# nrclaudio/spVIPES

Hardware: AMD Instinct MI355X
Metric: cells/sec/training-step (2-group PoE VAE) (higher is better)
Workload: dtype bf16

## Files before the change

### include/spvipes_hip.h

```cpp
#ifndef SPVIPES_HIP_H
#define SPVIPES_HIP_H

#include <stdint.h>

#ifdef __cplusplus
extern "C" {
#endif

#define SPV_OK 0
#define SPV_ERR_ARG (-1)
#define SPV_ERR_LAUNCH (-2)
#define SPV_ERR_UNSUPPORTED (-3)

#define SPV_COUNT_F32 0
#define SPV_COUNT_U16 1

#define SPV_NB_CMAX 64
#define SPV_DEC_KP 16
#define SPV_DEC_KS 32
#define SPV_DEC_KP_WIDE 32
#define SPV_DEC_KS_WIDE 64
#define SPV_DEC_CELLS_PER_WG 128

int spv_version(void);
// ... 266 lines not shown
typedef struct spv_linear_batch {
  spv_linear_prob p[SPV_MAXP];
  int32_t nprob, B;
  int32_t relu;
  float drop_p;
  uint64_t seed;
  const uint64_t* seed_ptr;
  int32_t accumulate;
} spv_linear_batch;
int spv_linear_fwd(const spv_linear_batch* a, void* stream);
int spv_linear_dgrad(const spv_linear_batch* a, void* stream);
int spv_linear_wgrad(const spv_linear_batch* a, float* wpart, int64_t wpart_elems, void* stream);

typedef struct spv_linear_pending_prob { float* dW; float* db; int32_t N, K; } spv_linear_pending_prob;
typedef struct spv_linear_pending {
  spv_linear_pending_prob p[SPV_MAXP];
  int32_t nprob;
  const float* wpart; int64_t prob_stride;
} spv_linear_pending;
int spv_linear_bwd(const spv_linear_batch* d, const spv_linear_batch* w, float* wpart, int64_t wpart_elems,
                   const spv_linear_pending* pending, void* stream);
int spv_linear_reduce_pending(const spv_linear_pending* pending, void* stream);

typedef struct spv_bn_prob {
  const float* X; int64_t ldx;
  float* Y; int64_t ldy;
  const float* gamma; const float* beta;
  float* running_mean; float* running_var;
  float* stats;
  float* part;
  const float* dY; int64_t lddy;
  float* dX; int64_t lddx;
  float* dgamma; float* dbeta;
  int32_t N;
  uint16_t* img_hi; uint16_t* img_lo; int64_t ld_img; int32_t img_rows;
} spv_bn_prob;
typedef struct spv_bn_batch {
  spv_bn_prob p[SPV_MAXP];
  int32_t nprob, B, training, relu;
  float eps, momentum;
} spv_bn_batch;
int spv_bn_fwd(const spv_bn_batch* a, void* stream);
int spv_bn_bwd(const spv_bn_batch* a, void* stream);

typedef struct spv_sample_prob {
  const float* post; int32_t n;
// ... 147 lines not shown
```

### spvipes_amd/_abi.py

```python
from __future__ import annotations

import ctypes as C
import os
from typing import NamedTuple, Optional

import torch

_HERE = os.path.dirname(os.path.abspath(__file__))
LIB_PATH = os.path.join(_HERE, "_lib", "libspvipes_hip.so")

SPV_COUNT_F32, SPV_COUNT_U16 = 0, 1
NB_CMAX, DEC_KP, DEC_KS, DEC_CELLS_PER_WG = 64, 16, 32, 128
DEC_KPS = DEC_KP + DEC_KS


class DecSlots(NamedTuple):
    kslots: int
    KP: int
    KS: int
    KPS: int


DEC_NARROW = DecSlots(0, DEC_KP, DEC_KS, DEC_KPS)
DEC_WIDE = DecSlots(1, 32, 64, 96)
# ... 284 lines not shown
    "spv_de_median_ws_bytes": (C.c_int64, [C.c_int32, C.c_int32]),
    "spv_count_stats": (C.c_int, [C.POINTER(SpvCountStatsArgs), C.c_void_p]),
    "spv_count_stats_partial": (C.c_int, [C.POINTER(SpvCountStatsArgs), C.c_void_p]),
    "spv_count_stats_merge": (C.c_int, [C.POINTER(SpvCountStatsArgs), C.c_void_p]),
    "spv_count_stats_tile": (C.c_int32, []),
    "spv_count_stats_slab": (C.c_int32, []),
    "spv_count_stats_ws_bytes": (C.c_int64, [C.c_int32, C.c_int32]),
    "spv_count_totals": (C.c_int, [C.POINTER(SpvCounts), C.c_int32, C.c_int32, C.c_void_p, C.c_void_p]),
    "spv_csr_totals": (C.c_int, [C.c_void_p, C.c_void_p, C.c_void_p, C.c_int32, C.c_int32, C.c_int32, C.c_void_p, C.c_void_p]),
    "spv_dec_dz": (C.c_int, [C.POINTER(SpvDecParams), C.c_void_p, C.c_void_p, C.c_void_p, C.c_void_p]),
    "spv_dec_softmax_bwd": (C.c_int, [C.POINTER(SpvDecParams), C.c_void_p, C.c_void_p, C.c_void_p, C.c_void_p]),
    "spv_dec_heads_bwd": (C.c_int, [C.POINTER(SpvDecParams), C.c_void_p, C.c_void_p, C.c_void_p, C.c_void_p, C.c_void_p]),
    "spv_dec_tables_grouped": (C.c_int, [C.POINTER(SpvDecGroup), C.c_int32, C.c_void_p]),
    "spv_dec_logits_grouped": (C.c_int, [C.POINTER(SpvDecGroup), C.c_int32, C.c_void_p]),
    "spv_dec_lse_grouped": (C.c_int, [C.POINTER(SpvDecGroup), C.c_int32, C.c_void_p]),
    "spv_dec_nb_fwd_grouped": (C.c_int, [C.POINTER(SpvDecGroup), C.c_int32, C.c_int32, C.c_void_p]),
    "spv_dec_heads_bwd_grouped": (C.c_int, [C.POINTER(SpvDecGroup), C.c_int32, C.c_void_p]),
    "spv_gemm_bf16_grouped": (C.c_int, [C.POINTER(SpvGemmArgs), C.c_int32, C.c_void_p]),
    "spv_linear_fwd": (C.c_int, [C.POINTER(SpvLinearBatch), C.c_void_p]),
    "spv_linear_dgrad": (C.c_int, [C.POINTER(SpvLinearBatch), C.c_void_p]),
    "spv_linear_wgrad": (C.c_int, [C.POINTER(SpvLinearBatch), C.c_void_p, C.c_int64, C.c_void_p]),
    "spv_linear_bwd": (C.c_int, [C.POINTER(SpvLinearBatch), C.POINTER(SpvLinearBatch), C.c_void_p, C.c_int64, C.POINTER(SpvLinearPending), C.c_void_p]),
    "spv_linear_reduce_pending": (C.c_int, [C.POINTER(SpvLinearPending), C.c_void_p]),
    "spv_bn_fwd": (C.c_int, [C.POINTER(SpvBnBatch), C.c_void_p]),
    "spv_bn_bwd": (C.c_int, [C.POINTER(SpvBnBatch), C.c_void_p]),
    "spv_enc_sample_fwd": (C.c_int, [C.POINTER(SpvSampleBatch), C.c_void_p]),
    "spv_enc_sample_bwd": (C.c_int, [C.POINTER(SpvSampleBatch), C.c_void_p]),
    "spv_enc_heads_fwd": (C.c_int, [C.POINTER(SpvBnBatch), C.POINTER(SpvSampleBatch), C.c_void_p]),
    "spv_enc_heads_bwd": (C.c_int, [C.POINTER(SpvBnBatch), C.POINTER(SpvSampleBatch), C.c_void_p]),
    "spv_poe_partner": (C.c_int, [C.c_void_p, C.c_void_p, C.c_int32, C.c_int32, C.c_void_p, C.c_void_p, C.c_void_p, C.c_void_p, C.c_void_p,
                                  C.c_void_p, C.c_void_p, C.c_void_p, C.c_void_p, C.c_void_p, C.c_void_p]),
    "spv_poe_rank": (C.c_int, [C.c_void_p, C.c_void_p, C.c_int32, C.c_int32, C.c_void_p, C.c_void_p, C.c_void_p, C.c_void_p, C.c_void_p, C.c_void_p, C.c_void_p]),
    "spv_poe_fuse_fwd": (C.c_int, [C.POINTER(SpvPoeArgs), C.c_void_p]),
    "spv_poe_fuse_bwd": (C.c_int, [C.POINTER(SpvPoeArgs), C.c_void_p]),
    "spv_plan_invmap": (C.c_int, [C.c_void_p, C.c_int32, C.c_void_p, C.c_int32, C.c_void_p, C.c_int32, C.c_void_p, C.c_int32, C.c_void_p]),
    "spv_plan_argmax": (C.c_int, [C.POINTER(SpvPlan), C.c_void_p, C.c_void_p, C.c_void_p, C.c_void_p, C.c_int32, C.c_int32, C.c_void_p,
                                  C.c_void_p, C.c_void_p]),
    "spv_plan_expert_fwd": (C.c_int, [C.POINTER(SpvPlanExpertArgs), C.c_void_p]),
    "spv_plan_expert_bwd": (C.c_int, [C.POINTER(SpvPlanExpertArgs), C.c_void_p]),
    "spv_poe_comp_fwd": (C.c_int, [C.POINTER(SpvPoeCompArgs), C.c_void_p]),
    "spv_poe_comp_bwd": (C.c_int, [C.POINTER(SpvPoeCompArgs), C.c_void_p]),
    "spv_zsplit_fwd": (C.c_int, [C.POINTER(SpvZsplitArgs), C.c_void_p]),
    "spv_zsplit_bwd": (C.c_int, [C.POINTER(SpvZsplitArgs), C.c_void_p]),
    "spv_bn_fold_fwd": (C.c_int, [C.POINTER(SpvFoldBatch), C.c_void_p]),
    "spv_bn_fold_bwd": (C.c_int, [C.POINTER(SpvFoldBatch), C.c_void_p]),
    "spv_trunk_fold_fwd": (C.c_int, [C.POINTER(SpvTrunkBatch), C.c_void_p]),
# ... 94 lines not shown
```

### spvipes_amd/csrc/spv_abi.hip

```cpp
#include "../../include/spvipes_hip.h"
#include "spv_common.h"
#include "spv_gemm.h"
#include "spv_fc1.h"
#include "spv_dec_gemm.h"
#include "spv_decoder.h"
#include "spv_dec_expected.h"
#include "spv_dec_sample.h"
#include "spv_de.h"
#include "spv_de_median.h"
#include "spv_count_stats.h"
#include "spv_small.h"
#include "spv_poe_n.h"

#include <cstdio>
#include <cstdlib>
#include <cstring>

using namespace spv;

static thread_local char g_err[512] = "";
static int fail(int code, const char* fmt, const char* what = "") {
  snprintf(g_err, sizeof(g_err), fmt, what);
  return code;
}
// ... 1224 lines not shown
  for (int i = 0; i < a->nprob; ++i)
    if (a->p[i].N <= 0 || a->p[i].K <= 0 || !a->p[i].W) return fail(SPV_ERR_ARG, "%s: bad problem", who);
  return SPV_OK;
}
static void linear_extents(const spv_linear_batch* a, int& nmax, int& kmax) {
  nmax = kmax = 0;
  for (int i = 0; i < a->nprob; ++i) { nmax = a->p[i].N > nmax ? a->p[i].N : nmax; kmax = a->p[i].K > kmax ? a->p[i].K : kmax; }
}

extern "C" int spv_linear_fwd(const spv_linear_batch* a, void* stream) {
  int rc = check_linear(a, "spv_linear_fwd");
  if (rc) return rc;
  for (int i = 0; i < a->nprob; ++i) if (!a->p[i].X || !a->p[i].Y) return fail(SPV_ERR_ARG, "spv_linear_fwd: null pointer%s");
  int nmax, kmax; linear_extents(a, nmax, kmax);
  int rows = a->B;
  for (int i = 0; i < a->nprob; ++i) {
    const spv_linear_prob& q = a->p[i];
    if (q.img_hi && (q.ld_img < q.N || q.img_rows < 0)) return fail(SPV_ERR_ARG, "spv_linear_fwd: bad operand image%s");
    if (q.img_hi && q.img_rows > rows) rows = q.img_rows;
  }
  hipLaunchKernelGGL(linear_fwd_kernel, dim3((rows + 63) / 64, (nmax + 63) / 64, a->nprob), dim3(256), 0, (hipStream_t)stream, *a);
  return launch_status("spv_linear_fwd");
}
extern "C" int spv_linear_dgrad(const spv_linear_batch* a, void* stream) {
  int rc = check_linear(a, "spv_linear_dgrad");
  if (rc) return rc;
  for (int i = 0; i < a->nprob; ++i)
    if (!a->p[i].dY || !a->p[i].dX || ((a->relu || a->drop_p > 0.f) && !a->p[i].Y)) return fail(SPV_ERR_ARG, "spv_linear_dgrad: null pointer%s");
  int nmax, kmax; linear_extents(a, nmax, kmax);
  hipLaunchKernelGGL(linear_dgrad_kernel, dim3((a->B + 63) / 64, (kmax + 63) / 64, a->nprob), dim3(256), 0, (hipStream_t)stream, *a);
  return launch_status("spv_linear_dgrad");
}
extern "C" int spv_linear_wgrad(const spv_linear_batch* a, float* wpart, int64_t wpart_elems, void* stream) {
  int rc = check_linear(a, "spv_linear_wgrad");
  if (rc) return rc;
  for (int i = 0; i < a->nprob; ++i)
    if (!a->p[i].dY || !a->p[i].X || !a->p[i].dW || ((a->relu || a->drop_p > 0.f) && !a->p[i].Y)) return fail(SPV_ERR_ARG, "spv_linear_wgrad: null pointer%s");
  if (!wpart) return fail(SPV_ERR_ARG, "spv_linear_wgrad: workspace missing%s");
  int nmax, kmax; linear_extents(a, nmax, kmax);
  const long prob_stride = (long)WG_SLICES * nmax * (kmax + 1);
  if (wpart_elems < prob_stride * a->nprob) return fail(SPV_ERR_ARG, "spv_linear_wgrad: workspace too small%s");
  hipStream_t s = (hipStream_t)stream;
  if (a->B <= WG_DIRECT_MAX_B) {
    hipLaunchKernelGGL(linear_wgrad_direct_kernel, dim3((nmax + 31) / 32, (kmax + 31) / 32, a->nprob), dim3(256), 0, s, *a);
    return launch_status("spv_linear_wgrad");
  }
// ... 49 lines not shown
    if (!wpart) return fail(SPV_ERR_ARG, "spv_linear_bwd: workspace missing%s");
    int nmax, kmax; linear_extents(w, nmax, kmax);
    prob_stride = (long)WG_SLICES * nmax * (kmax + 1);
    if (wpart_elems < prob_stride * w->nprob) return fail(SPV_ERR_ARG, "spv_linear_bwd: workspace too small%s");
    g.wgx = (nmax + 31) / 32; g.wgy = (kmax + 31) / 32;
    g.nw = g.wgx * g.wgy * w->nprob * (w->B <= WG_DIRECT_MAX_B ? 1 : WG_SLICES);
  }
  if (d && w && (d->B != w->B || (d->relu != 0) != (w->relu != 0) || d->drop_p != w->drop_p))
    return fail(SPV_ERR_ARG, "spv_linear_bwd: the two batches disagree in B / relu / drop_p%s");
  int nr = 0;
  if (pending) {
    int rc = check_pending(pending, "spv_linear_bwd", g.rgx);
    if (rc) return rc;
    if (w) {
      const float* pe = pending->wpart + pending->prob_stride * pending->nprob;
      if (wpart < pe && pending->wpart < wpart + wpart_elems) return fail(SPV_ERR_ARG, "spv_linear_bwd: wpart overlaps the pending workspace%s");
    }
    nr = g.rgx * pending->nprob;
  }
  static const spv_linear_pending no_pending = {};
  hipLaunchKernelGGL(linear_bwd_kernel, dim3((unsigned)(g.nd + g.nw + nr)), dim3(256), 0, (hipStream_t)stream, d ? *d : none, w ? *w : none,
                     pending ? *pending : no_pending, g, wpart, prob_stride);
  return launch_status("spv_linear_bwd");
}

static int check_bn(const spv_bn_batch* a, const char* who) {
  if (!a || a->nprob <= 0 || a->nprob > SPV_MAXP || a->B <= 0) return fail(SPV_ERR_ARG, "%s: bad batch", who);
  for (int i = 0; i < a->nprob; ++i) {
    const spv_bn_prob& q = a->p[i];
    if (q.N <= 0 || q.N > 256 || !q.X || !q.gamma || !q.beta || !q.running_mean || !q.running_var || !q.stats || !q.part)
      return fail(SPV_ERR_ARG, "%s: bad problem (N <= 256, non-null pointers)", who);
  }
  return SPV_OK;
}
static bool bn_all_narrow(const spv_bn_batch* a) {
  for (int i = 0; i < a->nprob; ++i) if (a->p[i].N > 64) return false;
  return true;
}
extern "C" int spv_bn_fwd(const spv_bn_batch* a, void* stream) {
  int rc = check_bn(a, "spv_bn_fwd");
  if (rc) return rc;
  for (int i = 0; i < a->nprob; ++i) if (!a->p[i].Y) return fail(SPV_ERR_ARG, "spv_bn_fwd: null output%s");
  dim3 grid((a->B + BN_ROWS - 1) / BN_ROWS, a->nprob);
  hipStream_t s = (hipStream_t)stream;
  int nmax = 0;
  for (int i = 0; i < a->nprob; ++i) nmax = a->p[i].N > nmax ? a->p[i].N : nmax;
// ... 882 lines not shown
```

### spvipes_amd/csrc/spv_small.h

```cpp
#pragma once
#include "../../include/spvipes_hip.h"
#include "spv_common.h"

namespace spv {


typedef spv_linear_prob LinearProb;
typedef spv_linear_batch LinearBatch;

__device__ __forceinline__ unsigned hash_u32(unsigned long long x) {
  x ^= x >> 33; x *= 0xff51afd7ed558ccdULL; x ^= x >> 33; x *= 0xc4ceb9fe1a85ec53ULL; x ^= x >> 33;
  return (unsigned)x;
}
__device__ __forceinline__ bool dropout_keep(unsigned long long seed, int prob, long idx, float p) {
  const unsigned key = ((unsigned)seed ^ ((unsigned)(seed >> 32) * 0x9E3779B9u)) + (unsigned)(prob + 1) * 0x85EBCA6Bu;
  unsigned x = (unsigned)idx * 747796405u + key;
  x = ((x >> ((x >> 28) + 4u)) ^ x) * 277803737u;
  x ^= x >> 22;
  x = x * 0x2C1B3C6Du + key;
  x ^= x >> 15;
  return (float)(x >> 8) * (1.0f / 16777216.0f) >= p;
}

__device__ __forceinline__ f16v mfma_f32(float x, float w, const f16v& c) { return __builtin_amdgcn_mfma_f32_32x32x2f32(x, w, c, 0, 0, 0); }
// ... 261 lines not shown
    else { if (vec) linear_dgrad_body<true, false>(d, prob, bx, by); else linear_dgrad_body<false, false>(d, prob, bx, by); }
    return;
  }
  bid -= g.nd;
  if (bid < g.nw) {
    const int bx = bid % g.wgx, by = (bid / g.wgx) % g.wgy, z = bid / (g.wgx * g.wgy);
    const bool masked = w.relu || w.drop_p > 0.f;
    if (w.B <= WG_DIRECT_MAX_B) {
      if (masked) linear_wgrad_body<true, true>(w, nullptr, 0, z, 0, bx, by, s_acc, s_b);
      else linear_wgrad_body<false, true>(w, nullptr, 0, z, 0, bx, by, s_acc, s_b);
    } else {
      const int prob = z / WG_SLICES, slice = z % WG_SLICES;
      if (masked) linear_wgrad_body<true, false>(w, wpart, prob_stride, prob, slice, bx, by, s_acc, s_b);
      else linear_wgrad_body<false, false>(w, wpart, prob_stride, prob, slice, bx, by, s_acc, s_b);
    }
    return;
  }
  bid -= g.nw;
  const int prob = bid / g.rgx;
  const spv_linear_pending_prob& t = pend.p[prob];
  linear_wgrad_reduce_body(t.dW, t.db, t.N, t.K, pend.wpart, pend.prob_stride, prob, bid % g.rgx);
}
static_assert(sizeof(LinearBatch) * 2 + sizeof(LinearPending) + sizeof(LinearBwdGrid) + 16 < 4096, "linear_bwd_kernel: kernel arguments must stay below 4096 bytes");

typedef spv_bn_prob BnProb;
typedef spv_bn_batch BnBatch;
constexpr int BN_ROWS = 32;

__device__ __forceinline__ int pow2_at_least(int n) { int p = 1; while (p < n) p <<= 1; return p; }

__global__ __launch_bounds__(256) void bn_stats_kernel(BnBatch a) {
  const BnProb& q = a.p[blockIdx.y];
  __shared__ float s_acc[256], s_mean[256];
  const int NC = pow2_at_least(q.N), RS = 256 / NC;
  const int c = threadIdx.x % NC, slot = threadIdx.x / NC;
  const int b0 = blockIdx.x * BN_ROWS, b1 = min(b0 + BN_ROWS, a.B);
  float s = 0.f;
  if (c < q.N) {
#pragma unroll 4
    for (int b = b0 + slot; b < b1; b += RS) s += q.X[(long)b * q.ldx + c];
  }
  s_acc[threadIdx.x] = s;
  __syncthreads();
  if (threadIdx.x < q.N) {
    float t = 0.f;
    for (int k = 0; k < RS; ++k) t += s_acc[k * NC + threadIdx.x];
// ... 1317 lines not shown
```

### spvipes_amd/nn_ops.py

```python
from __future__ import annotations

import ctypes as C
from typing import List, Optional, Sequence

import torch

from . import _abi
from ._abi import SpvBnBatch, SpvLinearBatch, SpvLinearPending, SpvSampleBatch, ptr, stream_ptr


def _lin_batch(B: int, relu: bool = False, drop_p: float = 0.0, seed=0, accumulate: bool = False) -> SpvLinearBatch:
    b = SpvLinearBatch()
    b.nprob, b.B, b.relu, b.drop_p, b.accumulate = 0, B, int(relu), float(drop_p), int(accumulate)
    if isinstance(seed, torch.Tensor):
        b.seed, b.seed_ptr = 0, seed.data_ptr()
    else:
        b.seed, b.seed_ptr = int(seed), None
    return b


def _add_lin(b: SpvLinearBatch, *, N: int, K: int, W=None, X=None, ldx=0, bias=None, Y=None, ldy=0, dY=None, lddy=0, dX=None, lddx=0,
             dW=None, db=None, keep=None, W2=None, n_w2=0) -> None:
    q = b.p[b.nprob]
    q.X, q.ldx, q.W, q.bias, q.Y, q.ldy, q.keep, q.W2, q.n_w2 = X, ldx, W, bias, Y, ldy, keep, W2, n_w2
# ... 21 lines not shown


def _linear_bwd(bd: Optional[SpvLinearBatch], bw: Optional[SpvLinearBatch], ws, key: str, pending: Optional[SpvLinearPending] = None) -> Optional[SpvLinearPending]:
    part, n, rec = None, 0, None
    if bw is not None:
        nmax = max(bw.p[i].N for i in range(bw.nprob))
        kmax = max(bw.p[i].K for i in range(bw.nprob))
        stride = _abi.WG_SLICES * nmax * (kmax + 1)
        n = bw.nprob * stride
        part = ws.get(key, (n,), torch.float32)
        if bw.B > _abi.WG_DIRECT_MAX_B:
            rec = SpvLinearPending()
            rec.nprob, rec.wpart, rec.prob_stride = bw.nprob, ptr(part), stride
            for i in range(bw.nprob):
                rec.p[i].dW, rec.p[i].db, rec.p[i].N, rec.p[i].K = bw.p[i].dW, bw.p[i].db, bw.p[i].N, bw.p[i].K
    _abi.call("spv_linear_bwd", C.byref(bd) if bd is not None else None, C.byref(bw) if bw is not None else None, ptr(part), n,
              C.byref(pending) if pending is not None else None, stream_ptr())
    return rec


def _reduce_pending(rec: Optional[SpvLinearPending]) -> None:
    if rec is not None:
        _abi.call("spv_linear_reduce_pending", C.byref(rec), stream_ptr())


def _fptr(t: torch.Tensor, col: int = 0) -> int:
    return t.data_ptr() + 4 * col


class EncoderSpec:

    def __init__(self, enc, h1_group: int, h1_col: int):
        self.enc, self.h1_group, self.h1_col = enc, h1_group, h1_col
        self.n = enc.n_topics

    def params(self) -> List[torch.Tensor]:
        e = self.enc
        return [e.fc2.weight, e.fc2.bias, e.mu_encoder[0].weight, e.mu_encoder[0].bias, e.lvar_encoder[0].weight, e.lvar_encoder[0].bias,
                e.mu_encoder[1].weight, e.mu_encoder[1].bias, e.lvar_encoder[1].weight, e.lvar_encoder[1].bias]


N_ENC_PARAMS = 10


class EncoderTails(torch.autograd.Function):

# ... 5 lines not shown
        par = [tensors[n_groups + i * N_ENC_PARAMS: n_groups + (i + 1) * N_ENC_PARAMS] for i in range(len(specs))]
        B, H = h1[0].shape[0], specs[0].enc.fc2.weight.shape[0]
        dev = h1[0].device
        for t in h1:
            if t.dtype != torch.float32 or not t.is_contiguous():
                raise _abi.SpvError("EncoderTails expects contiguous fp32 h1")
        new = lambda *s: torch.empty(*s, dtype=torch.float32, device=dev)
        h2 = [new(B, H) for _ in specs]
        pre = [new(B, 2 * s.n) for s in specs]
        post = [new(B, 2 * s.n) for s in specs]
        stats = [new(2, s.n, 2) for s in specs]
        nblk = -(-B // _abi.BN_ROWS)
        dp = float(drop_p) if training else 0.0
        b = _lin_batch(B, relu=True, drop_p=dp, seed=seed)
        keep_masks = []
        for i, (s, p, y) in enumerate(zip(specs, par, h2)):
            mk = None
            if masks is not None and masks[i] is not None and dp > 0:
                mk = masks[i].to(dev, torch.float32).contiguous()
                if mk.shape != (B, H):
                    raise _abi.SpvError("dropout mask must be [B, n_hidden]")
                keep_masks.append(mk)
            _add_lin(b, N=H, K=H, W=ptr(p[0]), bias=ptr(p[1]), X=_fptr(h1[s.h1_group], s.h1_col), ldx=h1[s.h1_group].shape[1], Y=ptr(y), ldy=H, keep=ptr(mk))
        _abi.call("spv_linear_fwd", C.byref(b), stream_ptr())
        b = _lin_batch(B)
        for s, p, x, y in zip(specs, par, h2, pre):
            _add_lin(b, N=s.n, K=H, W=ptr(p[2]), bias=ptr(p[3]), X=ptr(x), ldx=H, Y=_fptr(y, 0), ldy=2 * s.n)
            _add_lin(b, N=s.n, K=H, W=ptr(p[4]), bias=ptr(p[5]), X=ptr(x), ldx=H, Y=_fptr(y, s.n), ldy=2 * s.n)
        _abi.call("spv_linear_fwd", C.byref(b), stream_ptr())
        bn = SpvBnBatch()
        bn.nprob, bn.B, bn.training, bn.relu, bn.eps, bn.momentum = 0, B, int(training), 0, 1e-5, 0.1
        parts = []
        for s, p, x, y, st in zip(specs, par, pre, post, stats):
            for half, (g, be, mod) in enumerate(((p[6], p[7], s.enc.mu_encoder[1]), (p[8], p[9], s.enc.lvar_encoder[1]))):
                part = ws.get(f"tail_bn_part_{len(parts)}", (nblk, s.n, 2), torch.float32)
                parts.append(part)
                q = bn.p[bn.nprob]
                q.X, q.ldx, q.Y, q.ldy = _fptr(x, half * s.n), 2 * s.n, _fptr(y, half * s.n), 2 * s.n
                q.gamma, q.beta, q.running_mean, q.running_var = ptr(g), ptr(be), ptr(mod.running_mean), ptr(mod.running_var)
                q.stats, q.part, q.N = ptr(st[half]), ptr(part), s.n
                bn.nprob += 1
        scale = [new(B, s.n) for s in specs]
        logz = [new(B, s.n) for s in specs]
        theta = [new(B, s.n) for s in specs]
        kl = [new(B) for _ in specs]
        sb = SpvSampleBatch()
        sb.nprob, sb.B = len(specs), B
        for i, s in enumerate(specs):
            q = sb.p[i]
            q.post, q.n, q.eps, q.scale, q.logz, q.theta, q.kl = ptr(post[i]), s.n, ptr(eps[i].contiguous()), ptr(scale[i]), ptr(logz[i]), ptr(theta[i]), ptr(kl[i])
        _abi.call("spv_enc_heads_fwd", C.byref(bn), C.byref(sb), stream_ptr())
        ctx.specs, ctx.training, ctx.dp, ctx.seed, ctx.ws, ctx.n_groups, ctx.B, ctx.H = specs, training, dp, seed, ws, n_groups, B, H
# ... 53 lines not shown
                q.stats, q.part, q.N = ptr(stats[i][half]), ptr(ws.get(f"tail_bn_part_{k}", (nblk, s.n, 2), torch.float32)), s.n
                q.dY, q.lddy, q.dX, q.lddx = _fptr(d_post[i], half * s.n), 2 * s.n, _fptr(d_pre[i], half * s.n), 2 * s.n
                q.dgamma, q.dbeta = ptr(d_gb[i][2 * half]), ptr(d_gb[i][2 * half + 1])
                bn.nprob += 1
                k += 1
        if fused:
            _abi.call("spv_enc_heads_bwd", C.byref(bn), C.byref(sb), stream_ptr())
        else:
            _abi.call("spv_bn_bwd", C.byref(bn), stream_ptr())
        dWmu, dbmu, dWlv, dblv = ([pg[i][2][0] for i in range(E)], [pg[i][3][0] for i in range(E)], [pg[i][4][0] for i in range(E)], [pg[i][5][0] for i in range(E)])
        bwh = _lin_batch(B)
        for i, s in enumerate(specs):
            _add_lin(bwh, N=s.n, K=H, W=ptr(par[i][2]), X=ptr(h2[i]), ldx=H, dY=_fptr(d_pre[i], 0), lddy=2 * s.n, dW=ptr(dWmu[i]), db=ptr(dbmu[i]))
            _add_lin(bwh, N=s.n, K=H, W=ptr(par[i][4]), X=ptr(h2[i]), ldx=H, dY=_fptr(d_pre[i], s.n), lddy=2 * s.n, dW=ptr(dWlv[i]), db=ptr(dblv[i]))
        from . import ops as _ops
        wsw = ws if not isinstance(ws, (list, tuple)) else ws[0]
        one_launch = _ops.LINEAR_BWD
        if not one_launch:
            _wgrad(bwh, wsw)
        dh2 = [new(B, H) for _ in specs]
        b = _lin_batch(B)
        for i, s in enumerate(specs):
            _add_lin(b, N=2 * s.n, K=H, W=ptr(par[i][2]), W2=ptr(par[i][4]), n_w2=s.n, dY=ptr(d_pre[i]), lddy=2 * s.n, dX=ptr(dh2[i]), lddx=H)
        if one_launch:
            pend = _linear_bwd(b, bwh, wsw, "wgrad_part_heads")
        else:
            _abi.call("spv_linear_dgrad", C.byref(b), stream_ptr())
        dW2, db2 = [pg[i][0][0] for i in range(E)], [pg[i][1][0] for i in range(E)]
        covered = [sorted((s.h1_col, s.h1_col + H) for s in specs if s.h1_group == k) for k in range(n_groups)]
        full = [bool(c) and c[0][0] == 0 and c[-1][1] == h1[k].shape[1] and all(c[i][1] == c[i + 1][0] for i in range(len(c) - 1))
                for k, c in enumerate(covered)]
        dh1 = [torch.empty_like(t) if full[k] else torch.zeros_like(t) for k, t in enumerate(h1)]
        bw = _lin_batch(B, relu=True, drop_p=ctx.dp)
        bd = _lin_batch(B, relu=True, drop_p=ctx.dp)
        for i, s in enumerate(specs):
            x, ldx = _fptr(h1[s.h1_group], s.h1_col), h1[s.h1_group].shape[1]
            _add_lin(bw, N=H, K=H, W=ptr(par[i][0]), X=x, ldx=ldx, Y=ptr(h2[i]), ldy=H, dY=ptr(dh2[i]), lddy=H, dW=ptr(dW2[i]), db=ptr(db2[i]))
            _add_lin(bd, N=H, K=H, W=ptr(par[i][0]), Y=ptr(h2[i]), ldy=H, dY=ptr(dh2[i]), lddy=H, dX=_fptr(dh1[s.h1_group], s.h1_col), lddx=ldx)
        if one_launch:
            _reduce_pending(_linear_bwd(bd, bw, wsw, "wgrad_part_fc2", pend))
        else:
            _wgrad(bw, wsw)
            _abi.call("spv_linear_dgrad", C.byref(bd), stream_ptr())
        grads: List[Optional[torch.Tensor]] = list(dh1)
        for i in range(E):
            grads += [pg[i][j][1] for j in range(N_ENC_PARAMS)]
        return (None, None, None, None, None, None, None, *grads)


def _loc_logvar_block(loc: torch.Tensor, logvar: torch.Tensor):
    n = loc.shape[1]
    if (loc.dtype == torch.float32 and loc.stride(1) == 1 and logvar.stride(1) == 1 and loc.stride(0) == logvar.stride(0)
            and logvar.data_ptr() == loc.data_ptr() + 4 * n and loc.stride(0) >= 2 * n):
        return loc, loc.data_ptr(), loc.stride(0)
    blk = torch.cat([loc, logvar], dim=1).contiguous()
    return blk, blk.data_ptr(), 2 * n


def label_partners(labels: Sequence[torch.Tensor], ws):
    dev = labels[0].device
    lab = [l.flatten().contiguous().float() for l in labels]
    Bs = [lab[0].numel(), lab[1].numel()]
# ... 291 lines not shown
```

### spvipes_amd/ops.py

```python
from __future__ import annotations

import ctypes as C
import os
from dataclasses import dataclass
from typing import Dict, Optional, Tuple

import torch

from . import _abi
from ._abi import DEC_CELLS_PER_WG, NB_CMAX, SpvCounts, SpvDecParams, check, ptr, round_up, stream_ptr

N_HIDDEN_MIX = 256


@dataclass
class GroupCounts:

    X: torch.Tensor
    G: int
    col_off: int = 0
    resident: bool = False

    def __post_init__(self):
        self._xb = None
# ... 239 lines not shown
    return LABEL_PRE if LABEL_PRE >= 0 else (2 if B >= LABEL_PRE_MIN_B else 0)



DEC_PAIR = os.environ.get("SPV_DEC_PAIR", "auto")


def dec_pair_for(B: int, n_groups: int) -> bool:
    if n_groups != 2 or DEC_PAIR == "0":
        return False
    return True if DEC_PAIR == "1" else _SMALL_STEP


FC1_PAIR_SPLITS = os.environ.get("SPV_FC1_PAIR_SPLITS", "1") != "0"
DEC_PAIR_SPLITS = os.environ.get("SPV_DEC_PAIR_SPLITS", "1") != "0"
HEADS_DMA = os.environ.get("SPV_HEADS_DMA", "1") != "0"
FUSED_HEADS = os.environ.get("SPV_FUSED_HEADS", "1") != "0"
GSPLIT_WANT = int(os.environ.get("SPV_GSPLIT_WANT", "512"))
FUSED_HEADS_F32 = os.environ.get("SPV_FUSED_HEADS_F32", "1") != "0"
FUSED_DZ = os.environ.get("SPV_FUSED_DZ", "1") != "0"
FUSED_DZ_F32 = os.environ.get("SPV_FUSED_DZ_F32", "1") != "0"
DA_FIXUP = os.environ.get("SPV_DA_FIXUP", "0")
LINEAR_BWD = os.environ.get("SPV_LINEAR_BWD", "1") != "0"
TRUNK_FOLD = os.environ.get("SPV_TRUNK_FOLD", "1") != "0"
FUSED_PACK = os.environ.get("SPV_FUSED_PACK", "1") != "0"
DEFER_WM = os.environ.get("SPV_DEFER_WM", "1") != "0"
DEFER_BC = os.environ.get("SPV_DEFER_BC", "1") != "0"
DZ_ONLY = os.environ.get("SPV_DZ_ONLY", "0") != "0"
FWD_GROUP_STREAMS = os.environ.get("SPV_FWD_GROUP_STREAMS", "1") != "0"
BWD_GROUP_STREAMS = os.environ.get("SPV_BWD_GROUP_STREAMS", "1") != "0"
_PENDING: list = []
_PENDING_KEEP: list = []


def defer(stream, keep=()) -> None:
    if stream not in _PENDING:
        _PENDING.append(stream)
    _PENDING_KEEP.extend(keep)


def join_all_side_streams(device) -> None:
    dev = torch.device(device)
    cur = torch.cuda.current_stream(dev)
    capturing = torch.cuda.is_current_stream_capturing()
    for (idx, _i), st in _SIDE_STREAMS.items():
        if idx != dev.index or st is cur:
# ... 276 lines not shown
```

Measured before the change: 6.378 million.

## Fuse encoder fc2 and mu/logvar heads into one tail kernel

Adds a fused encoder-tail forward kernel that computes fc2 (with bias, relu and dropout) into shared memory and then runs both small head GEMMs from that staged tile in the same launch. This removes one launch and the global round trip of h2 before the heads read it. It also adds an optional fused backward chain (heads dgrad into fc2 dgrad, with head wgrad in the same grid and fc2 wgrad on a side stream), but that path is off by default. The trade-off is limited parallelism: each block covers only 64 rows, and the kernel is restricted to H up to 128.

Result: no change. 6.419 million, median of 2 (+0.6%).

```diff
diff --git a/include/spvipes_hip.h b/include/spvipes_hip.h
--- a/include/spvipes_hip.h
+++ b/include/spvipes_hip.h
@@ -312,6 +312,13 @@
                    const spv_linear_pending* pending, void* stream);
 int spv_linear_reduce_pending(const spv_linear_pending* pending, void* stream);
 
+int spv_enc_tail_fwd_supported(const spv_linear_batch* fc2, const spv_linear_batch* heads);
+int spv_enc_tail_fwd(const spv_linear_batch* fc2, const spv_linear_batch* heads, void* stream);
+
+int spv_enc_tail_bwd_supported(const spv_linear_batch* dheads, const spv_linear_batch* dfc2);
+int spv_enc_tail_bwd(const spv_linear_batch* dheads, const spv_linear_batch* dfc2, const spv_linear_batch* wheads, float* wpart,
+                     int64_t wpart_elems, void* stream);
+
 typedef struct spv_bn_prob {
   const float* X; int64_t ldx;
   float* Y; int64_t ldy;
diff --git a/spvipes_amd/_abi.py b/spvipes_amd/_abi.py
--- a/spvipes_amd/_abi.py
+++ b/spvipes_amd/_abi.py
@@ -330,6 +330,10 @@
     "spv_linear_wgrad": (C.c_int, [C.POINTER(SpvLinearBatch), C.c_void_p, C.c_int64, C.c_void_p]),
     "spv_linear_bwd": (C.c_int, [C.POINTER(SpvLinearBatch), C.POINTER(SpvLinearBatch), C.c_void_p, C.c_int64, C.POINTER(SpvLinearPending), C.c_void_p]),
     "spv_linear_reduce_pending": (C.c_int, [C.POINTER(SpvLinearPending), C.c_void_p]),
+    "spv_enc_tail_fwd_supported": (C.c_int, [C.POINTER(SpvLinearBatch), C.POINTER(SpvLinearBatch)]),
+    "spv_enc_tail_fwd": (C.c_int, [C.POINTER(SpvLinearBatch), C.POINTER(SpvLinearBatch), C.c_void_p]),
+    "spv_enc_tail_bwd_supported": (C.c_int, [C.POINTER(SpvLinearBatch), C.POINTER(SpvLinearBatch)]),
+    "spv_enc_tail_bwd": (C.c_int, [C.POINTER(SpvLinearBatch), C.POINTER(SpvLinearBatch), C.POINTER(SpvLinearBatch), C.c_void_p, C.c_int64, C.c_void_p]),
     "spv_bn_fwd": (C.c_int, [C.POINTER(SpvBnBatch), C.c_void_p]),
     "spv_bn_bwd": (C.c_int, [C.POINTER(SpvBnBatch), C.c_void_p]),
     "spv_enc_sample_fwd": (C.c_int, [C.POINTER(SpvSampleBatch), C.c_void_p]),
diff --git a/spvipes_amd/csrc/spv_abi.hip b/spvipes_amd/csrc/spv_abi.hip
--- a/spvipes_amd/csrc/spv_abi.hip
+++ b/spvipes_amd/csrc/spv_abi.hip
@@ -1270,6 +1270,48 @@
   hipLaunchKernelGGL(linear_fwd_kernel, dim3((rows + 63) / 64, (nmax + 63) / 64, a->nprob), dim3(256), 0, (hipStream_t)stream, *a);
   return launch_status("spv_linear_fwd");
 }
+static bool is_aligned16(const void* p) { return (reinterpret_cast<uintptr_t>(p) & 15) == 0; }
+static int enc_tail_fwd_shape_ok(const spv_linear_batch* fc2, const spv_linear_batch* heads) {
+  if (heads->nprob != 2 * fc2->nprob || heads->B != fc2->B || heads->relu || heads->drop_p > 0.f) return 0;
+  const int H = fc2->p[0].N;
+  if (H % 64 != 0 || H > ENC_TAIL_HMAX) return 0;
+  for (int e = 0; e < fc2->nprob; ++e) {
+    const spv_linear_prob& q = fc2->p[e];
+    if (q.N != H || q.K != H || q.img_hi || (q.ldx & 3) || !is_aligned16(q.X) || !is_aligned16(q.W)) return 0;
+    for (int k = 0; k < 2; ++k) {
+      const spv_linear_prob& t = heads->p[2 * e + k];
+      if (t.N > 32 || t.K != H || t.X != q.Y || t.ldx != q.ldy || t.img_hi || t.keep || !is_aligned16(t.W)) return 0;
+    }
+  }
+  return 1;
+}
+extern "C" int spv_enc_tail_fwd_supported(const spv_linear_batch* fc2, const spv_linear_batch* heads) {
+  if (check_linear(fc2, "spv_enc_tail_fwd_supported") || check_linear(heads, "spv_enc_tail_fwd_supported")) return 0;
+  return enc_tail_fwd_shape_ok(fc2, heads);
+}
+extern "C" int spv_enc_tail_fwd(const spv_linear_batch* fc2, const spv_linear_batch* heads, void* stream) {
+  int rc = check_linear(fc2, "spv_enc_tail_fwd");
+  if (rc) return rc;
+  rc = check_linear(heads, "spv_enc_tail_fwd");
+  if (rc) return rc;
+  for (int i = 0; i < fc2->nprob; ++i) if (!fc2->p[i].X || !fc2->p[i].Y) return fail(SPV_ERR_ARG, "spv_enc_tail_fwd: null pointer%s");
+  for (int i = 0; i < heads->nprob; ++i) if (!heads->p[i].X || !heads->p[i].Y) return fail(SPV_ERR_ARG, "spv_enc_tail_fwd: null pointer%s");
+  if (!enc_tail_fwd_shape_ok(fc2, heads))
+    return fail(SPV_ERR_ARG, "spv_enc_tail_fwd: shapes outside the fused kernel (ask spv_enc_tail_fwd_supported; run two spv_linear_fwd launches)%s");
+  EncTailFwdArgs a = {};
+  a.B = fc2->B; a.H = fc2->p[0].N; a.relu = fc2->relu; a.drop_p = fc2->drop_p; a.seed = fc2->seed; a.seed_ptr = (const unsigned long long*)fc2->seed_ptr;
+  for (int e = 0; e < fc2->nprob; ++e) {
+    const spv_linear_prob& q = fc2->p[e];
+    EncTailFwdProb& t = a.p[e];
+    t.X = q.X; t.ldx = q.ldx; t.W = q.W; t.bias = q.bias; t.Y = q.Y; t.ldy = q.ldy; t.keep = q.keep;
+    for (int k = 0; k < 2; ++k) {
+      const spv_linear_prob& hq = heads->p[2 * e + k];
+      t.Wh[k] = hq.W; t.bh[k] = hq.bias; t.P[k] = hq.Y; t.ldp[k] = hq.ldy; t.n[k] = hq.N;
+    }
+  }
+  hipLaunchKernelGGL(enc_tail_fwd_kernel, dim3((a.B + 63) / 64, fc2->nprob), dim3(64 * 2 * (a.H / 32)), 0, (hipStream_t)stream, a);
+  return launch_status("spv_enc_tail_fwd");
+}
 extern "C" int spv_linear_dgrad(const spv_linear_batch* a, void* stream) {
   int rc = check_linear(a, "spv_linear_dgrad");
   if (rc) return rc;
@@ -1365,6 +1407,62 @@
   hipLaunchKernelGGL(linear_bwd_kernel, dim3((unsigned)(g.nd + g.nw + nr)), dim3(256), 0, (hipStream_t)stream, d ? *d : none, w ? *w : none,
                      pending ? *pending : no_pending, g, wpart, prob_stride);
   return launch_status("spv_linear_bwd");
+}
+
+static int enc_tail_bwd_shape_ok(const spv_linear_batch* dheads, const spv_linear_batch* dfc2) {
+  if (dheads->nprob != dfc2->nprob || dheads->B != dfc2->B || dheads->relu || dheads->drop_p > 0.f || dheads->accumulate || dfc2->accumulate) return 0;
+  const int H = dfc2->p[0].N;
+  if (H % 64 != 0 || H > ENC_TAIL_HMAX) return 0;
+  const bool masked = dfc2->relu || dfc2->drop_p > 0.f;
+  for (int e = 0; e < dfc2->nprob; ++e) {
+    const spv_linear_prob& q = dfc2->p[e];
+    const spv_linear_prob& t = dheads->p[e];
+    if (q.N != H || q.K != H || q.W2 || !q.dY || !q.dX || (masked && !q.Y)) return 0;
+    if (t.K != H || t.N > 64 || !t.dY || t.dX != q.dY || t.lddx != q.lddy || (t.W2 && (t.n_w2 <= 0 || t.n_w2 > t.N))) return 0;
+  }
+  return 1;
+}
+extern "C" int spv_enc_tail_bwd_supported(const spv_linear_batch* dheads, const spv_linear_batch* dfc2) {
+  if (check_linear(dheads, "spv_enc_tail_bwd_supported") || check_linear(dfc2, "spv_enc_tail_bwd_supported")) return 0;
+  return enc_tail_bwd_shape_ok(dheads, dfc2);
+}
+extern "C" int spv_enc_tail_bwd(const spv_linear_batch* dheads, const spv_linear_batch* dfc2, const spv_linear_batch* wheads, float* wpart,
+                                int64_t wpart_elems, void* stream) {
+  int rc = check_linear(dheads, "spv_enc_tail_bwd");
+  if (rc) return rc;
+  rc = check_linear(dfc2, "spv_enc_tail_bwd");
+  if (rc) return rc;
+  if (!enc_tail_bwd_shape_ok(dheads, dfc2))
+    return fail(SPV_ERR_ARG, "spv_enc_tail_bwd: shapes outside the fused kernel (ask spv_enc_tail_bwd_supported; run the spv_linear_bwd launches)%s");
+  EncTailBwdArgs a = {};
+  a.B = dfc2->B; a.H = dfc2->p[0].N; a.drop_p = dfc2->drop_p;
+  a.nbx = (a.B + 63) / 64; a.nchain = a.nbx * dfc2->nprob;
+  const bool masked = dfc2->relu || dfc2->drop_p > 0.f;
+  for (int e = 0; e < dfc2->nprob; ++e) {
+    const spv_linear_prob& q = dfc2->p[e];
+    const spv_linear_prob& t = dheads->p[e];
+    EncTailBwdProb& o = a.p[e];
+    o.dP = t.dY; o.lddp = t.lddy; o.N = t.N; o.nw2 = t.n_w2; o.Wh = t.W; o.Wh2 = t.W2;
+    o.dY = t.dX; o.lddy = t.lddx; o.Y = masked ? q.Y : nullptr; o.ldy = q.ldy; o.W = q.W; o.dX = q.dX; o.lddx = q.lddx;
+  }
+  static const spv_linear_batch none = {};
+  long prob_stride = 0;
+  if (wheads) {
+    rc = check_linear(wheads, "spv_enc_tail_bwd");
+    if (rc) return rc;
+    if (wheads->B != a.B || wheads->relu || wheads->drop_p > 0.f || wheads->accumulate) return fail(SPV_ERR_ARG, "spv_enc_tail_bwd: bad weight-gradient batch%s");
+    for (int i = 0; i < wheads->nprob; ++i)
+      if (!wheads->p[i].dY || !wheads->p[i].X || !wheads->p[i].dW) return fail(SPV_ERR_ARG, "spv_enc_tail_bwd: null pointer%s");
+    if (!wpart) return fail(SPV_ERR_ARG, "spv_enc_tail_bwd: workspace missing%s");
+    int nmax, kmax; linear_extents(wheads, nmax, kmax);
+    prob_stride = (long)WG_SLICES * nmax * (kmax + 1);
+    if (wpart_elems < prob_stride * wheads->nprob) return fail(SPV_ERR_ARG, "spv_enc_tail_bwd: workspace too small%s");
+    a.wgx = (nmax + 31) / 32; a.wgy = (kmax + 31) / 32;
+    a.nw = a.wgx * a.wgy * wheads->nprob * (a.B <= WG_DIRECT_MAX_B ? 1 : WG_SLICES);
+  }
+  hipLaunchKernelGGL(enc_tail_bwd_kernel, dim3((unsigned)(a.nchain + a.nw)), dim3(64 * 2 * (a.H / 32)), 0, (hipStream_t)stream, a,
+                     wheads ? *wheads : none, wpart, prob_stride);
+  return launch_status("spv_enc_tail_bwd");
 }
 
 static int check_bn(const spv_bn_batch* a, const char* who) {
diff --git a/spvipes_amd/csrc/spv_small.h b/spvipes_amd/csrc/spv_small.h
--- a/spvipes_amd/csrc/spv_small.h
+++ b/spvipes_amd/csrc/spv_small.h
@@ -307,6 +307,206 @@
   linear_wgrad_reduce_body(t.dW, t.db, t.N, t.K, pend.wpart, pend.prob_stride, prob, bid % g.rgx);
 }
 static_assert(sizeof(LinearBatch) * 2 + sizeof(LinearPending) + sizeof(LinearBwdGrid) + 16 < 4096, "linear_bwd_kernel: kernel arguments must stay below 4096 bytes");
+
+constexpr int ENC_TAIL_HMAX = 128, ENC_TAIL_PAD = 4;
+struct EncTailFwdProb {
+  const float* X; long ldx;
+  const float* W; const float* bias;
+  float* Y; long ldy;
+  const float* keep;
+  const float* Wh[2]; const float* bh[2]; float* P[2]; long ldp[2]; int n[2];
+};
+struct EncTailFwdArgs {
+  EncTailFwdProb p[SPV_MAXP];
+  int B, H, relu; float drop_p;
+  unsigned long long seed; const unsigned long long* seed_ptr;
+};
+static_assert(sizeof(EncTailFwdArgs) < 4096, "enc_tail_fwd_kernel: kernel arguments must stay below 4096 bytes");
+
+__global__ __launch_bounds__(512) void enc_tail_fwd_kernel(EncTailFwdArgs a) {
+  __shared__ __attribute__((aligned(16))) float s_h[64 * (ENC_TAIL_HMAX + ENC_TAIL_PAD)];
+  const EncTailFwdProb& q = a.p[blockIdx.y];
+  const int H = a.H, LP = H + ENC_TAIL_PAD;
+  const int lane = threadIdx.x & 63, wave = threadIdx.x >> 6, nwaves = blockDim.x >> 6, h = lane >> 5, r = lane & 31;
+  const int rb = 32 * (wave & 1), n0 = 32 * (wave >> 1);
+  const int b0 = blockIdx.x * 64 + rb;
+  if (b0 < a.B) {
+    const int row = b0 + r, col = n0 + r;
+    const float* xr = q.X + (long)min(row, a.B - 1) * q.ldx;
+    const float* wr = q.W + (long)col * H;
+    const float bias_v = *(q.bias ? q.bias + col : q.W);
+    const float bias = q.bias ? bias_v : 0.f;
+    const unsigned long long seed_v = *(a.seed_ptr ? a.seed_ptr : reinterpret_cast<const unsigned long long*>(q.W));
+    const unsigned long long seed = a.seed + (a.seed_ptr ? seed_v : 0ull);
+    f16v acc;
+#pragma unroll
+    for (int i = 0; i < 16; ++i) acc[i] = 0.f;
+    float xa[8], wb[8];
+    load8<true>(xr + 8 * h, xr, H - 8 * h, xa);
+    load8<true>(wr + 8 * h, wr, H - 8 * h, wb);
+    for (int k0 = 0; k0 < H; k0 += 16) {
+      float xn[8], wn[8];
+      const int kn = k0 + 16 + 8 * h;
+      load8<true>(xr + kn, xr, H - kn, xn);
+      load8<true>(wr + kn, wr, H - kn, wn);
+#pragma unroll
+      for (int j = 0; j < 8; ++j) acc = mfma_f32(xa[j], wb[j], acc);
+#pragma unroll
+      for (int j = 0; j < 8; ++j) { xa[j] = xn[j]; wb[j] = wn[j]; }
+    }
+#pragma unroll
+    for (int i = 0; i < 16; ++i) {
+      const int rl = rb + crow(i, h), b = blockIdx.x * 64 + rl;
+      float v = acc[i] + bias;
+      if (a.relu) v = fmaxf(v, 0.f);
+      if (a.drop_p > 0.f) {
+        const int bm = min(b, a.B - 1);
+        const bool keep = q.keep ? (q.keep[(long)bm * H + col] != 0.f) : dropout_keep(seed, blockIdx.y, (long)b * H + col, a.drop_p);
+        v = keep ? v * (1.0f / (1.0f - a.drop_p)) : 0.f;
+      }
+      s_h[rl * LP + col] = v;
+      if (b < a.B) q.Y[(long)b * q.ldy + col] = v;
+    }
+  }
+  __syncthreads();
+  for (int t = wave; t < 4; t += nwaves) {
+    const int hd = t >> 1, rbh = 32 * (t & 1), bh0 = blockIdx.x * 64 + rbh;
+    if (bh0 >= a.B) continue;
+    const int n = q.n[hd];
+    const float* xs = s_h + (rbh + r) * LP;
+    const float* wr = q.Wh[hd] + (long)min(r, n - 1) * H;
+    const float bias_v = *(q.bh[hd] ? q.bh[hd] + min(r, n - 1) : q.Wh[hd]);
+    const float bias = q.bh[hd] ? bias_v : 0.f;
+    f16v acc;
+#pragma unroll
+    for (int i = 0; i < 16; ++i) acc[i] = 0.f;
+    float xa[8], wb[8];
+    load8<true>(xs + 8 * h, xs, H - 8 * h, xa);
+    load8<true>(wr + 8 * h, wr, H - 8 * h, wb);
+    for (int k0 = 0; k0 < H; k0 += 16) {
+      float xn[8], wn[8];
+      const int kn = k0 + 16 + 8 * h;
+      load8<true>(xs + kn, xs, H - kn, xn);
+      load8<true>(wr + kn, wr, H - kn, wn);
+#pragma unroll
+      for (int j = 0; j < 8; ++j) acc = mfma_f32(xa[j], wb[j], acc);
+#pragma unroll
+      for (int j = 0; j < 8; ++j) { xa[j] = xn[j]; wb[j] = wn[j]; }
+    }
+    if (r >= n) continue;
+#pragma unroll
+    for (int i = 0; i < 16; ++i) {
+      const int b = bh0 + crow(i, h);
+      if (b < a.B) q.P[hd][(long)b * q.ldp[hd] + r] = acc[i] + bias;
+    }
+  }
+}
+
+struct EncTailBwdProb {
+  const float* dP; long lddp; int N, nw2;
+  const float* Wh; const float* Wh2;
+  float* dY; long lddy;
+  const float* Y; long ldy;
+  const float* W;
+  float* dX; long lddx;
+};
+struct EncTailBwdArgs {
+  EncTailBwdProb p[SPV_MAXP];
+  int B, H, nbx, nchain, nw, wgx, wgy; float drop_p;
+};
+static_assert(sizeof(EncTailBwdArgs) + sizeof(LinearBatch) + 32 < 4096, "enc_tail_bwd_kernel: kernel arguments must stay below 4096 bytes");
+
+template <bool VEC>
+__device__ __forceinline__ void tail_dgrad_fetch(const float* gr, const float* wc, const float* wc2, int n, int N, int nw2, int K, float (&g)[8], float (&w)[8]) {
+  load8<VEC>(gr + n, gr, N - n, g);
+#pragma unroll
+  for (int j = 0; j < 8; ++j) {
+    const int r = n + j;
+    const bool ok = r < N;
+    const float t = *((r < nw2) ? wc + (long)(ok ? r : 0) * K : wc2 + (long)(ok ? r - nw2 : 0) * K);
+    w[j] = ok ? t : 0.f;
+  }
+}
+template <bool VEC>
+__device__ __forceinline__ void enc_tail_bwd_chain(const EncTailBwdArgs& a, int prob, int bx, float* s_g) {
+  const EncTailBwdProb& q = a.p[prob];
+  const int H = a.H, LP = H + ENC_TAIL_PAD;
+  const int lane = threadIdx.x & 63, wave = threadIdx.x >> 6, h = lane >> 5, r = lane & 31;
+  const int rb = 32 * (wave & 1), k0 = 32 * (wave >> 1);
+  const int b0 = bx * 64 + rb, col = k0 + r;
+  const bool live = b0 < a.B;
+  const float sc = (a.drop_p > 0.f) ? 1.0f / (1.0f - a.drop_p) : 1.0f;
+  if (live) {
+    const float* gr = q.dP + (long)min(b0 + r, a.B - 1) * q.lddp;
+    const float* wc = q.Wh + col;
+    const float* wc2 = (q.Wh2 ? q.Wh2 : q.Wh) + col;
+    const int nw2 = q.Wh2 ? q.nw2 : q.N;
+    float y[16];
+    const float* yb = q.Y ? q.Y : q.Wh;
+    const long ldy = q.Y ? q.ldy : 0;
+#pragma unroll
+    for (int i = 0; i < 16; ++i) y[i] = yb[(long)min(b0 + crow(i, h), a.B - 1) * ldy + (q.Y ? col : 0)];
+    f16v acc;
+#pragma unroll
+    for (int i = 0; i < 16; ++i) acc[i] = 0.f;
+    float ga[8], wb[8];
+    tail_dgrad_fetch<VEC>(gr, wc, wc2, 8 * h, q.N, nw2, H, ga, wb);
+    for (int n0 = 0; n0 < q.N; n0 += 16) {
+      float gn[8], wn[8];
+      tail_dgrad_fetch<VEC>(gr, wc, wc2, n0 + 16 + 8 * h, q.N, nw2, H, gn, wn);
+#pragma unroll
+      for (int j = 0; j < 8; ++j) acc = mfma_f32(ga[j], wb[j], acc);
+#pragma unroll
+      for (int j = 0; j < 8; ++j) { ga[j] = gn[j]; wb[j] = wn[j]; }
+    }
+#pragma unroll
+    for (int i = 0; i < 16; ++i) {
+      const int rl = rb + crow(i, h), b = bx * 64 + rl;
+      if (b < a.B) q.dY[(long)b * q.lddy + col] = acc[i];
+      s_g[rl * LP + col] = q.Y ? ((y[i] > 0.f) ? acc[i] * sc : 0.f) : acc[i];
+    }
+  }
+  __syncthreads();
+  if (!live) return;
+  const float* gs = s_g + (rb + r) * LP;
+  const float* wc = q.W + col;
+  f16v acc;
+#pragma unroll
+  for (int i = 0; i < 16; ++i) acc[i] = 0.f;
+  float ga[8], wb[8];
+  tail_dgrad_fetch<true>(gs, wc, wc, 8 * h, H, H, H, ga, wb);
+  for (int n0 = 0; n0 < H; n0 += 16) {
+    float gn[8], wn[8];
+    tail_dgrad_fetch<true>(gs, wc, wc, n0 + 16 + 8 * h, H, H, H, gn, wn);
+#pragma unroll
+    for (int j = 0; j < 8; ++j) acc = mfma_f32(ga[j], wb[j], acc);
+#pragma unroll
+    for (int j = 0; j < 8; ++j) { ga[j] = gn[j]; wb[j] = wn[j]; }
+  }
+#pragma unroll
+  for (int i = 0; i < 16; ++i) {
+    const int b = b0 + crow(i, h);
+    if (b < a.B) q.dX[(long)b * q.lddx + col] = acc[i];
+  }
+}
+
+__global__ __launch_bounds__(512) void enc_tail_bwd_kernel(EncTailBwdArgs a, LinearBatch w, float* wpart, long prob_stride) {
+  __shared__ __attribute__((aligned(16))) float s_g[64 * (ENC_TAIL_HMAX + ENC_TAIL_PAD)];
+  __shared__ float s_acc[3][16][64], s_b[3][32];
+  int bid = blockIdx.x;
+  if (bid < a.nchain) {
+    const int prob = bid / a.nbx, bx = bid % a.nbx;
+    const EncTailBwdProb& q = a.p[prob];
+    const bool vec = ((q.lddp & 3) == 0) && aligned16(q.dP) && ((q.N & 7) == 0);
+    if (vec) enc_tail_bwd_chain<true>(a, prob, bx, s_g); else enc_tail_bwd_chain<false>(a, prob, bx, s_g);
+    return;
+  }
+  if (threadIdx.x >= 256) return;
+  bid -= a.nchain;
+  const int bx = bid % a.wgx, by = (bid / a.wgx) % a.wgy, z = bid / (a.wgx * a.wgy);
+  if (w.B <= WG_DIRECT_MAX_B) linear_wgrad_body<false, true>(w, nullptr, 0, z, 0, bx, by, s_acc, s_b);
+  else linear_wgrad_body<false, false>(w, wpart, prob_stride, z / WG_SLICES, z % WG_SLICES, bx, by, s_acc, s_b);
+}
 
 typedef spv_bn_prob BnProb;
 typedef spv_bn_batch BnBatch;
diff --git a/spvipes_amd/nn_ops.py b/spvipes_amd/nn_ops.py
--- a/spvipes_amd/nn_ops.py
+++ b/spvipes_amd/nn_ops.py
@@ -67,6 +67,47 @@
 def _reduce_pending(rec: Optional[SpvLinearPending]) -> None:
     if rec is not None:
         _abi.call("spv_linear_reduce_pending", C.byref(rec), stream_ptr())
+
+
+def _tail_fwd(fc2: SpvLinearBatch, heads: SpvLinearBatch) -> None:
+    from . import ops as _ops
+    if _ops.ENC_TAIL and _abi.load().spv_enc_tail_fwd_supported(C.byref(fc2), C.byref(heads)):
+        _abi.call("spv_enc_tail_fwd", C.byref(fc2), C.byref(heads), stream_ptr())
+    else:
+        _abi.call("spv_linear_fwd", C.byref(fc2), stream_ptr())
+        _abi.call("spv_linear_fwd", C.byref(heads), stream_ptr())
+
+
+def _tail_bwd(bdh: SpvLinearBatch, bd2: SpvLinearBatch, bwh: SpvLinearBatch, ws, key: str) -> Optional[SpvLinearPending]:
+    nmax = max(bwh.p[i].N for i in range(bwh.nprob))
+    kmax = max(bwh.p[i].K for i in range(bwh.nprob))
+    stride = _abi.WG_SLICES * nmax * (kmax + 1)
+    n = bwh.nprob * stride
+    part = ws.get(key, (n,), torch.float32)
+    rec = None
+    if bwh.B > _abi.WG_DIRECT_MAX_B:
+        rec = SpvLinearPending()
+        rec.nprob, rec.wpart, rec.prob_stride = bwh.nprob, ptr(part), stride
+        for i in range(bwh.nprob):
+            rec.p[i].dW, rec.p[i].db, rec.p[i].N, rec.p[i].K = bwh.p[i].dW, bwh.p[i].db, bwh.p[i].N, bwh.p[i].K
+    _abi.call("spv_enc_tail_bwd", C.byref(bdh), C.byref(bd2), C.byref(bwh), ptr(part), n, stream_ptr())
+    return rec
+
+
+def _tail_wgrad_off_chain(bw: SpvLinearBatch, ws, pend: Optional[SpvLinearPending], dev, keep) -> None:
+    from . import ops as _ops
+    cur = torch.cuda.current_stream(dev)
+    side = _ops.group_streams(dev)[1] if _ops.ENC_TAIL_WGRAD != "inline" else cur
+    if side is cur:
+        _reduce_pending(_linear_bwd(None, bw, ws, "wgrad_part_fc2", pend))
+        return
+    side.wait_stream(cur)
+    with torch.cuda.stream(side):
+        _reduce_pending(_linear_bwd(None, bw, ws, "wgrad_part_fc2", pend))
+    if _ops.DEFER_JOIN:
+        _ops.defer(side, keep)
+    else:
+        cur.wait_stream(side)
 
 
 def _fptr(t: torch.Tensor, col: int = 0) -> int:
@@ -118,12 +159,11 @@
                     raise _abi.SpvError("dropout mask must be [B, n_hidden]")
                 keep_masks.append(mk)
             _add_lin(b, N=H, K=H, W=ptr(p[0]), bias=ptr(p[1]), X=_fptr(h1[s.h1_group], s.h1_col), ldx=h1[s.h1_group].shape[1], Y=ptr(y), ldy=H, keep=ptr(mk))
-        _abi.call("spv_linear_fwd", C.byref(b), stream_ptr())
-        b = _lin_batch(B)
+        bh = _lin_batch(B)
         for s, p, x, y in zip(specs, par, h2, pre):
-            _add_lin(b, N=s.n, K=H, W=ptr(p[2]), bias=ptr(p[3]), X=ptr(x), ldx=H, Y=_fptr(y, 0), ldy=2 * s.n)
-            _add_lin(b, N=s.n, K=H, W=ptr(p[4]), bias=ptr(p[5]), X=ptr(x), ldx=H, Y=_fptr(y, s.n), ldy=2 * s.n)
-        _abi.call("spv_linear_fwd", C.byref(b), stream_ptr())
+            _add_lin(bh, N=s.n, K=H, W=ptr(p[2]), bias=ptr(p[3]), X=ptr(x), ldx=H, Y=_fptr(y, 0), ldy=2 * s.n)
+            _add_lin(bh, N=s.n, K=H, W=ptr(p[4]), bias=ptr(p[5]), X=ptr(x), ldx=H, Y=_fptr(y, s.n), ldy=2 * s.n)
+        _tail_fwd(b, bh)
         bn = SpvBnBatch()
         bn.nprob, bn.B, bn.training, bn.relu, bn.eps, bn.momentum = 0, B, int(training), 0, 1e-5, 0.1
         parts = []
@@ -223,10 +263,11 @@
         b = _lin_batch(B)
         for i, s in enumerate(specs):
             _add_lin(b, N=2 * s.n, K=H, W=ptr(par[i][2]), W2=ptr(par[i][4]), n_w2=s.n, dY=ptr(d_pre[i]), lddy=2 * s.n, dX=ptr(dh2[i]), lddx=H)
-        if one_launch:
+        want_fused = bool(one_launch and _ops.ENC_TAIL and _ops.ENC_TAIL_BWD)
+        if not one_launch:
+            _abi.call("spv_linear_dgrad", C.byref(b), stream_ptr())
+        elif not want_fused:
             pend = _linear_bwd(b, bwh, wsw, "wgrad_part_heads")
-        else:
-            _abi.call("spv_linear_dgrad", C.byref(b), stream_ptr())
         dW2, db2 = [pg[i][0][0] for i in range(E)], [pg[i][1][0] for i in range(E)]
         covered = [sorted((s.h1_col, s.h1_col + H) for s in specs if s.h1_group == k) for k in range(n_groups)]
         full = [bool(c) and c[0][0] == 0 and c[-1][1] == h1[k].shape[1] and all(c[i][1] == c[i + 1][0] for i in range(len(c) - 1))
@@ -238,7 +279,13 @@
             x, ldx = _fptr(h1[s.h1_group], s.h1_col), h1[s.h1_group].shape[1]
             _add_lin(bw, N=H, K=H, W=ptr(par[i][0]), X=x, ldx=ldx, Y=ptr(h2[i]), ldy=H, dY=ptr(dh2[i]), lddy=H, dW=ptr(dW2[i]), db=ptr(db2[i]))
             _add_lin(bd, N=H, K=H, W=ptr(par[i][0]), Y=ptr(h2[i]), ldy=H, dY=ptr(dh2[i]), lddy=H, dX=_fptr(dh1[s.h1_group], s.h1_col), lddx=ldx)
-        if one_launch:
+        fused_chain = want_fused and bool(_abi.load().spv_enc_tail_bwd_supported(C.byref(b), C.byref(bd)))
+        if fused_chain:
+            pend = _tail_bwd(b, bd, bwh, wsw, "wgrad_part_heads")
+            _tail_wgrad_off_chain(bw, wsw, pend, dev, keep=[*dh2, *h2, *h1, *d_pre, *dW2, *db2, *dWmu, *dbmu, *dWlv, *dblv])
+        elif one_launch:
+            if want_fused:
+                pend = _linear_bwd(b, bwh, wsw, "wgrad_part_heads")
             _reduce_pending(_linear_bwd(bd, bw, wsw, "wgrad_part_fc2", pend))
         else:
             _wgrad(bw, wsw)
diff --git a/spvipes_amd/ops.py b/spvipes_amd/ops.py
--- a/spvipes_amd/ops.py
+++ b/spvipes_amd/ops.py
@@ -285,6 +285,9 @@
 FUSED_DZ_F32 = os.environ.get("SPV_FUSED_DZ_F32", "1") != "0"
 DA_FIXUP = os.environ.get("SPV_DA_FIXUP", "0")
 LINEAR_BWD = os.environ.get("SPV_LINEAR_BWD", "1") != "0"
+ENC_TAIL = os.environ.get("SPV_ENC_TAIL", "1") != "0"
+ENC_TAIL_BWD = os.environ.get("SPV_ENC_TAIL_BWD", "0") != "0"
+ENC_TAIL_WGRAD = os.environ.get("SPV_ENC_TAIL_WGRAD", "side")
 TRUNK_FOLD = os.environ.get("SPV_TRUNK_FOLD", "1") != "0"
 FUSED_PACK = os.environ.get("SPV_FUSED_PACK", "1") != "0"
 DEFER_WM = os.environ.get("SPV_DEFER_WM", "1") != "0"
```
